# scalar-labs/jepsen

Measured on AMD Instinct MI355X. Metric: history ops verified/sec (node), independent cas-register 10k keys, 1/2/4/8 GPU, higher is better.
Workload: dtype int64

## Files before the change

### include/jh.h

```cpp
#ifndef JH_H
#define JH_H

#include <stddef.h>
#include <stdint.h>

#ifdef __cplusplus
extern "C" {
#endif

#define JH_ABI_VERSION 8

#define JH_OK            0
#define JH_EINVAL        1
#define JH_EUNSUPPORTED  2
#define JH_EDEVICE       3
#define JH_ENOMEM        4

#define JH_TYPE_INVOKE 0
#define JH_TYPE_OK     1
#define JH_TYPE_FAIL   2
#define JH_TYPE_INFO   3

#define JH_F_READ  0
#define JH_F_WRITE 1
// ... 48 lines not shown
#define JH_LIN_INTERN_PER_KEY  4
#define JH_LIN_NO_HELPERS      8
#define JH_LIN_HELPERS_NOW    16
#define JH_LIN_PHASE1_ONLY    32
#define JH_LIN_SKIP_PHASE1    64
#define JH_LIN_NO_HANDOVER   128
#define JH_LIN_STREAM        256
#define JH_LIN_NO_RESUME     512
#define JH_LIN_EXACT_COUNT  1024
#define JH_EXPLORED_UNCOUNTED (-3)
#define JH_LIN_NO_SPEC      2048
#define JH_LIN_SPEC_FIRST   4096
#define JH_LIN_HELP_STALL   8192
#define JH_LIN_NO_TAKEOVER  16384
#define JH_LIN_TAKEOVER     32768

typedef struct jh_lin_opts {
    int64_t init_value;
    int64_t budget;
    int64_t stream;
    int32_t algorithm;
    int32_t flags;
    int64_t quick_budget;
    int64_t phase2_budget;
    int32_t helpers;
    int32_t helper_late_us;
    int32_t xw_waves;
    int32_t p2_waves_per_cu;
    int32_t lean_waves;
    int32_t wide_waves;
    int32_t handover_min;
    int32_t p1_waves_per_cu;
    int32_t bfs_wgs;
    int32_t helper_stall_min;
} jh_lin_opts;

#define JH_DEFAULT_BUDGET (1 << 20)

typedef struct jh_key_verdict {
    int32_t valid;
    int32_t cause;
    int64_t fail_entry;
    int64_t explored;
    int64_t previous_ok;
    int64_t last_op;
    int32_t analyzer;
    int32_t reserved;
} jh_key_verdict;

// ... 29 lines not shown
    int64_t lean_entries;
    int64_t wide_entries;
    int64_t xw_entries;
    int64_t waves[4];
    int64_t streamed;
    int64_t p3_entries;
    double  p2_start_ms;
    double  p1_span_ms;
    int64_t resumed;
    int64_t resume_bytes;
    int64_t spec_jobs;
    int64_t spec_dead;
    int64_t spec_merges;
    int64_t spec_nodes;
    int64_t takeovers;
} jh_summary;

typedef struct jh_ctx jh_ctx;

int  jh_version(void);
int  jh_open(int device, jh_ctx **out);
int  jh_open_multi(int n_gpus, jh_ctx **out);
int  jh_open_devices(const int32_t *devices, int n, jh_ctx **out);
int  jh_n_devices(const jh_ctx *ctx);
void jh_close(jh_ctx *ctx);

int  jh_key_costs(const jh_history *h, int64_t *cost , char *err, size_t errlen);

int jh_check_cas_independent(jh_ctx *ctx, const jh_history *h,
                             const jh_lin_opts *opts,
// ... 258 lines not shown
```

### jepsen_amd/_abi.py

```python
import ctypes as C

JH_ABI_VERSION = 8

JH_OK, JH_EINVAL, JH_EUNSUPPORTED, JH_EDEVICE, JH_ENOMEM = 0, 1, 2, 3, 4
TYPE_INVOKE, TYPE_OK, TYPE_FAIL, TYPE_INFO = 0, 1, 2, 3
F_READ, F_WRITE, F_CAS, F_ADD = 0, 1, 2, 3
F_ENQUEUE, F_DEQUEUE, F_DRAIN = 4, 5, 6
F_FIRST_INTERNED = 16
NIL = -(1 << 63)

VALID, UNKNOWN, INVALID = 0, 1, 2

CAUSES = {
    0: None,
    1: "budget",
    2: "window",
    3: "double-invoke",
    4: "orphan-completion",
    5: "unsupported-f",
    6: "nil-value",
    7: "overflow",
    8: "states",
    9: "deferred",
    10: "multiple-writes",
# ... 25 lines not shown

ALGO_COMPETITION, ALGO_WGL, ALGO_LINEAR = 0, 1, 2
ALGORITHMS = {"competition": ALGO_COMPETITION, "wgl": ALGO_WGL, "linear": ALGO_LINEAR}
LIN_BFS_ONLY, LIN_GEN_JUMP, LIN_INTERN_PER_KEY, LIN_NO_HELPERS, LIN_HELPERS_NOW = 1, 2, 4, 8, 16
LIN_PHASE1_ONLY, LIN_SKIP_PHASE1 = 32, 64
LIN_NO_HANDOVER = 128
LIN_STREAM = 256
LIN_NO_RESUME = 512
LIN_EXACT_COUNT = 1024
EXPLORED_UNCOUNTED = -3
LIN_NO_SPEC = 2048
LIN_SPEC_FIRST = 4096
LIN_HELP_STALL = 8192
LIN_NO_TAKEOVER = 16384
LIN_TAKEOVER = 32768
CAUSE_DEFERRED = 9


class JhLinOpts(C.Structure):
    _fields_ = [("init_value", C.c_int64), ("budget", C.c_int64), ("stream", C.c_int64),
                ("algorithm", C.c_int32), ("flags", C.c_int32),
                ("quick_budget", C.c_int64), ("phase2_budget", C.c_int64),
                ("helpers", C.c_int32), ("helper_late_us", C.c_int32),
                ("xw_waves", C.c_int32), ("p2_waves_per_cu", C.c_int32),
                ("lean_waves", C.c_int32), ("wide_waves", C.c_int32),
                ("handover_min", C.c_int32), ("p1_waves_per_cu", C.c_int32),
                ("bfs_wgs", C.c_int32), ("helper_stall_min", C.c_int32)]


VERDICT_FIELDS = ("valid", "cause", "fail_entry", "explored", "previous_ok", "last_op", "analyzer")
ANALYZER_WGL, ANALYZER_LINEAR = 0, 1
ANALYZERS = {ANALYZER_WGL: "wgl", ANALYZER_LINEAR: "linear"}


class JhKeyVerdict(C.Structure):
    _fields_ = [("valid", C.c_int32), ("cause", C.c_int32),
                ("fail_entry", C.c_int64), ("explored", C.c_int64),
                ("previous_ok", C.c_int64), ("last_op", C.c_int64),
                ("analyzer", C.c_int32), ("reserved", C.c_int32)]


class JhSummary(C.Structure):
    _fields_ = [("valid", C.c_int64), ("n_invalid", C.c_int64), ("n_unknown", C.c_int64),
                ("first_fail_entry", C.c_int64), ("n_keys", C.c_int64),
                ("explored", C.c_int64), ("memo_probes", C.c_int64),
                ("device_ms", C.c_double), ("dfs_ms", C.c_double),
                ("seq_ms", C.c_double), ("bfs_ms", C.c_double), ("n_deferred", C.c_int64),
                ("deferred_entries", C.c_int64), ("seq_probes", C.c_int64),
                ("p3_ms", C.c_double), ("wide_ms", C.c_double), ("xw_ms", C.c_double),
                ("p3_probes", C.c_int64), ("wide_probes", C.c_int64), ("xw_probes", C.c_int64),
                ("helper_probes", C.c_int64), ("n_deferred_wide", C.c_int64), ("n_phase3", C.c_int64),
                ("n_phase3_wide", C.c_int64), ("n_xw", C.c_int64), ("lean_entries", C.c_int64),
                ("wide_entries", C.c_int64), ("xw_entries", C.c_int64), ("waves", C.c_int64 * 4),
                ("streamed", C.c_int64), ("p3_entries", C.c_int64), ("p2_start_ms", C.c_double),
                ("p1_span_ms", C.c_double),
                ("resumed", C.c_int64), ("resume_bytes", C.c_int64),
                ("spec_jobs", C.c_int64), ("spec_dead", C.c_int64), ("spec_merges", C.c_int64),
                ("spec_nodes", C.c_int64), ("takeovers", C.c_int64)]


class JhLinConfig(C.Structure):
    _fields_ = [("key", C.c_int64), ("model_value", C.c_int64), ("n_linearized", C.c_int32),
                ("n_pending", C.c_int32), ("rows_off", C.c_int64),
                ("last_row", C.c_int64)]


CONFIGS_PER_KEY = 10


class JhSetResult(C.Structure):
    _fields_ = [("valid", C.c_int32), ("cause", C.c_int32),
                ("attempt_count", C.c_int64), ("acknowledged_count", C.c_int64),
                ("ok_count", C.c_int64), ("lost_count", C.c_int64),
# ... 187 lines not shown
```

### jepsen_amd/_native.py

```python
import ctypes as C
import os
import threading

import numpy as np

from . import _abi as A

_HERE = os.path.dirname(os.path.abspath(__file__))
LIB_PATH = os.environ.get("JH_LIB") or os.path.join(_HERE, "libjh.so")
_lib = None
_lock = threading.Lock()


class JhError(RuntimeError):
    def __init__(self, code, msg):
        super().__init__(f"libjh error {code}: {msg}")
        self.code = code
        self.msg = msg


def lib():
    global _lib
    with _lock:
        if _lib is None:
# ... 99 lines not shown

def _opts(init, budget, stream=0, algorithm=None, exact_count=True, **tune):
    o = A.JhLinOpts()
    o.init_value = A.NIL if init is None else int(init)
    o.budget = int(budget or 0)
    o.stream = int(stream)
    if isinstance(algorithm, str):
        algorithm = A.ALGORITHMS[algorithm]
    o.algorithm = int(algorithm or 0)
    for k, v in tune.items():
        if k not in dict(A.JhLinOpts._fields_) or k in ("init_value", "budget", "stream", "algorithm", "reserved"):
            raise TypeError(f"unknown jh_lin_opts field {k}")
        setattr(o, k, int(v))
    if exact_count:
        o.flags |= A.LIN_EXACT_COUNT
    return o


def key_costs(cols):
    h = A.make_history(cols)
    out = np.zeros(max(cols.n_keys, 1), dtype=np.int64)
    err = C.create_string_buffer(256)
    rc = lib().jh_key_costs(C.byref(h), out.ctypes.data_as(C.POINTER(C.c_int64)), err, len(err))
    _raise(rc, err)
    return out[:cols.n_keys]


class HostBuffer:

    def __init__(self, count, dtype):
# ... 393 lines not shown
```

### jepsen_amd/csrc/jh_api.hip

```cpp
#include "jh_internal.h"
#include <algorithm>
#include <unordered_map>
#include <vector>

static void set_err(char *err, size_t errlen, const std::string &msg) {
    if (!err || errlen == 0) return;
    size_t k = std::min(errlen - 1, msg.size());
    memcpy(err, msg.data(), k);
    err[k] = 0;
}

template <class F>
static int guarded(char *err, size_t errlen, F &&f) {
    try {
        f();
        set_err(err, errlen, "");
        return JH_OK;
    } catch (const JhException &e) {
        set_err(err, errlen, e.msg);
        return e.code;
    } catch (const std::exception &e) {
        set_err(err, errlen, std::string("internal error: ") + e.what());
        return JH_EDEVICE;
    }
// ... 123 lines not shown
        char e[512] = "";
        int rc = guarded(e, sizeof e, [&] { check_hist(h); });
        if (rc == JH_OK) rc = multi_check_cas_independent(ctx, h, opts, out, sum, e, sizeof e);
        set_err(err, errlen, e);
        return rc;
    }
    std::lock_guard<std::mutex> g(ctx->mu);
    return guarded(err, errlen, [&] {
        check_hist(h);
        HIP_TRY(hipSetDevice(ctx->device));
        hipStream_t st = ctx->stream;
        jh_history d = stage_history(ctx, h, true, false);
        const int64_t K = h->n_keys;
        jh_key_verdict *dv = ctx->ws<jh_key_verdict>(WS_VERDICT, std::max<int64_t>(K, 1));
        if (K == 0) {
            if (sum) { memset(sum, 0, sizeof *sum); sum->first_fail_entry = -1; }
            return;
        }
        lin_check_independent(ctx, &d, opts, true, dv, sum, st);
        HIP_TRY(hipMemcpyAsync(out, dv, sizeof(jh_key_verdict) * K, hipMemcpyDeviceToHost, st));
        HIP_TRY(hipStreamSynchronize(st));
    });
}

int jh_check_cas_independent_device(jh_ctx *ctx, const jh_history *h, const jh_lin_opts *opts,
                                    jh_key_verdict *out_dev, jh_summary *sum, char *err,
                                    size_t errlen) {
    if (!ctx || !out_dev) { set_err(err, errlen, "null context or output"); return JH_EINVAL; }
    ctx = primary(ctx);
    std::lock_guard<std::mutex> g(ctx->mu);
    return guarded(err, errlen, [&] {
        check_hist(h);
        if (!h->on_device) throw_jh(JH_EINVAL, "jh_check_cas_independent_device needs on_device=1");
        HIP_TRY(hipSetDevice(ctx->device));
        hipStream_t st = opts && opts->stream ? (hipStream_t)(intptr_t)opts->stream : ctx->stream;
        if (h->n_keys == 0) {
            if (sum) { memset(sum, 0, sizeof *sum); sum->first_fail_entry = -1; }
            return;
        }
        lin_check_independent(ctx, h, opts, true, out_dev, sum, st);
    });
}

__global__ void k_cfg_slots(const int64_t *__restrict__ keys, int n, int64_t K, int32_t *slot) {
    const int i = blockIdx.x * blockDim.x + threadIdx.x;
    if (i < n && keys[i] >= 0 && keys[i] < K) slot[keys[i]] = i;
}

struct NoopRead { int64_t call, ret; };
static std::vector<std::vector<NoopRead>> noop_reads(const jh_history *h, bool keyed, const int64_t *keys, int nq) {
    const int64_t n = h->n;
    std::vector<int64_t> pr, ty, fc, va, ke;
// ... 397 lines not shown
```

### jepsen_amd/csrc/jh_internal.h

```cpp
#pragma once
#include <hip/hip_runtime.h>
#include <cstdint>
#include <cstdio>
#include <cstdlib>
#include <cstring>
#include <mutex>
#include <thread>
#include <vector>
#include <string>
#include "../../include/jh.h"

#define JH_WAVE 64

struct JhError {
    int code = JH_OK;
    std::string msg;
};

#define HIP_TRY(expr)                                                                 \
    do {                                                                              \
        hipError_t _e = (expr);                                                       \
        if (_e != hipSuccess) {                                                       \
            throw_hip(_e, #expr, __FILE__, __LINE__);                                 \
        }                                                                             \
// ... 86 lines not shown
    WS_SPEC, WS_SPEC_RES, WS_DEBUG_WG, WS_HANDOFF, WS_RS_LOG2,
    WS_U_META, WS_U_PART, WS_U_LIST, WS_U_ALT, WS_U_ALT2, WS_U_BITS, WS_U_TMP, WS_U_FLAG, WS_U_RUNS, WS_U_PAIRS,
    WS_U_CNT, WS_U_IDX, WS_U_SEL, WS_U_OUT,
    WS_B_META, WS_B_WORDS, WS_B_TCNT, WS_B_TBASE, WS_B_TMP, WS_B_ROW, WS_B_START, WS_B_CNT, WS_B_OFF, WS_B_TOT,
    WS_B_BAD, WS_B_CLS, WS_B_FIRST, WS_B_PARTS, WS_B_ACC, WS_B_OUT, WS_B_TRI,
    WS_LF_META, WS_LF_WORDS, WS_LF_TCNT, WS_LF_TBASE, WS_LF_TMP, WS_LF_ROW, WS_LF_START, WS_LF_CNT, WS_LF_GRP, WS_LF_MASK,
    WS_LF_WKEY, WS_LF_WROW, WS_LF_FIRST, WS_LF_KEYS, WS_LF_IDX, WS_LF_RANK, WS_LF_SLOT, WS_LF_CTAB, WS_LF_VTAB, WS_LF_GBITS,
    WS_LF_FLAG, WS_LF_SKEY, WS_LF_SMASK, WS_LF_SROW, WS_LF_PC, WS_LF_OUT,
    WS_CR_META, WS_CR_WORDS, WS_CR_TCNT, WS_CR_TBASE, WS_CR_TMP, WS_CR_WKEY, WS_CR_WVAL, WS_CR_RKEY, WS_CR_RPERM, WS_CR_RROW,
    WS_CR_OFF, WS_CR_TIER, WS_CR_KV, WS_CR_EXP, WS_CR_MISS, WS_CR_SOFF, WS_CR_SCRATCH, WS_CR_OUT, WS_CR_SEG, WS_CR_MBUF,
    WS_CY_META, WS_CY_TMP, WS_CY_PKEY, WS_CY_PROW, WS_CY_COMP, WS_CY_REV, WS_CY_IP, WS_CY_ICOMP, WS_CY_CNT,
    WS_CY_TXN, WS_CY_REC, WS_CY_HASH, WS_CY_HIDX, WS_CY_RAW, WS_CY_EDGES, WS_CY_REACH, WS_CY_BS, WS_CY_REG, WS_CY_SEL,
    WS_CY_FWD, WS_CY_BWD, WS_CY_CSR, WS_CY_STATE, WS_CY_LABEL, WS_CY_SIZE, WS_CY_KEYS, WS_CY_VALS,
    WS_CY_AP_META, WS_CY_AP_ROWS, WS_CY_AP_RECS, WS_CY_AP_LONGEST,
    WS_CY_MO_META, WS_CY_MO_ROWS, WS_CY_MO_RECS,
    WS_COUNT
};

__device__ __forceinline__ uint64_t jh_mix64(uint64_t x) {
    x ^= x >> 33; x *= 0xff51afd7ed558ccdULL;
    x ^= x >> 33; x *= 0xc4ceb9fe1a85ec53ULL;
    x ^= x >> 33; return x;
}

template <class T, class Op>
__device__ __forceinline__ T block_reduce256(T v, Op op, T *sh ) {
    for (int o = 32; o > 0; o >>= 1) v = op(v, (T)__shfl_xor(v, o));
    __syncthreads();
    if ((threadIdx.x & 63) == 0) sh[threadIdx.x >> 6] = v;
    __syncthreads();
// ... 11 lines not shown
    return (int)g;
}

jh_history stage_history(jh_ctx *ctx, const jh_history *h, bool need_key, bool need_aux);
bool ingest_columns(jh_ctx *ctx, const int64_t *const src[7], int64_t *const dst[7], int64_t n, hipStream_t st);
void ingest_free(struct Ingest *g);

struct LinCfgReq {
    const int64_t *keys_dev;
    int32_t n_q, per_key;
    const int32_t *slot_dev;
    jh_lin_config *out_dev;
    int32_t *n_dev;
    int64_t *rows_dev;
};
void lin_check_independent(jh_ctx *ctx, const jh_history *dh, const jh_lin_opts *opts,
                           bool keyed, jh_key_verdict *out_dev, jh_summary *sum,
                           hipStream_t stream, const LinCfgReq *cfg = nullptr);
void key_index(jh_ctx *ctx, const jh_history *dh, int64_t *key_off, int64_t *rows, hipStream_t stream);
void counter_check(jh_ctx *ctx, const jh_history *dh, int64_t *reads_out, int64_t reads_cap,
                   int64_t *n_reads, int64_t *n_errors, int64_t *first_err, int32_t *valid,
                   int32_t *cause, hipStream_t stream);
void set_check(jh_ctx *ctx, const jh_history *dh, jh_set_result *res, int64_t *runs[4],
               int64_t runs_cap, hipStream_t stream);
void set_check_bitmaps(jh_ctx *ctx, const jh_history *dh, jh_set_result *res, uint32_t *bits_out[4],
                       int64_t words_cap, int64_t *base, int64_t *n_words, hipStream_t stream);
void set_full_check(jh_ctx *ctx, const jh_history *dh, const int64_t *time_dev, bool linearizable, int64_t read_batch,
                    jh_set_full_result *res, int64_t *lists_out[3], int64_t list_cap, hipStream_t stream);
void total_queue_check(jh_ctx *ctx, const jh_history *dh, jh_queue_result *res, int64_t *outs[4],
                       int64_t cap, hipStream_t stream);
// ... 33 lines not shown
```

### jepsen_amd/csrc/jh_lin.hip

```cpp
#include "jh_internal.h"
#include <hipcub/hipcub.hpp>
#include <algorithm>
#include <type_traits>
#include "lin/lin_common.h"

namespace {

constexpr int F_READ = 0, F_WRITE = 1, F_CAS = 2, F_OTHER = 4;
constexpr int T_INVOKE = 0, T_OK = 1, T_FAIL = 2, T_INFO = 3;
constexpr uint64_t VIOL_NONE = ~0ULL;
#ifndef JH_LDS_TBL
#define JH_LDS_TBL 0
#endif
constexpr int LDS_TBL = JH_LDS_TBL;
#ifdef JH_STEP_PROF
#define PROF_MARK(v) const unsigned long long v = __builtin_amdgcn_s_memtime()
#define PROF_ADD(acc, a, b) acc += (b) - (a)
#else
#define PROF_MARK(v)
#define PROF_ADD(acc, a, b)
#endif
#ifdef JH_DFS_STATS
#define DFS_STAT(x) x
#else
// ... 334 lines not shown
}
__device__ __forceinline__ bool handover(const DfsArgs &A, uint32_t ins) {
    if (A.handover_min <= 0 || ins < (uint32_t)A.handover_min) return false;
    int q = 0;
    if ((threadIdx.x & 63) == 0) q = __hip_atomic_load(A.queue, __ATOMIC_RELAXED, __HIP_MEMORY_SCOPE_AGENT);
    q = __builtin_amdgcn_readlane(q, 0);
    return q >= (A.n_list_dev ? *A.n_list_dev : A.n_list);
}
constexpr int64_t P2_BUDGET = 1 << 16;
constexpr int64_t QUICK_BUDGET = 8192;
constexpr int32_t HANDOVER_MIN = 1024;
constexpr int32_t P1_PRIO_INS = 0;
constexpr int HELPERS = 64;
constexpr uint64_t HELPER_LATE_US = 250;
constexpr uint32_t HELPER_STALL_MIN = 4096;
constexpr int HELPER_MAINS = 32;

__device__ __forceinline__ bool emit_verdict(jh_key_verdict *out, int32_t *claim, int key,
                                             const jh_key_verdict &v) {
    if (claim && atomicCAS(&claim[key], 0, 1) != 0) return false;
    out[key] = v;
    return true;
}

__device__ __forceinline__ uint64_t ballot(bool b) { return __ballot(b); }
__device__ __forceinline__ int mbcnt(uint64_t m) {
    return __builtin_amdgcn_mbcnt_hi((uint32_t)(m >> 32), __builtin_amdgcn_mbcnt_lo((uint32_t)m, 0));
}
__device__ __forceinline__ int rfl(int x) { return __builtin_amdgcn_readfirstlane(x); }
__device__ __forceinline__ uint32_t rflu(uint32_t x) { return (uint32_t)__builtin_amdgcn_readfirstlane((int)x); }
// ... 3300 lines not shown
    uint32_t *tmp;
    uint64_t *tmpk;
    int32_t linear;
    const int32_t *cfg_slot;
    jh_lin_config *cfg_out;
    int32_t *cfg_n;
    int64_t *cfg_rows;
    int32_t cfg_per;
    const int64_t *col_val, *col_val2;
    int64_t vmin, init_value;
    int32_t per_key_values;
    const int32_t *live_n;
    const int32_t *p1_done, *p1_tot;
    unsigned long long *t_span;
    unsigned long long *tl;
};

struct BfsShared {
    KeyInfo K;
    jh_key_verdict v;
    int key, need, maxw, status, mode, gclear, ovf, term;
    unsigned npend, npend2, nfront, nnext, tmax, lcount, r;
    unsigned nnodes, nostore, dlen, clen, cnext, ok;
    unsigned fbase;
    unsigned long long count, ccount, plen;
    alignas(16) uint32_t win_vv[64];
    uint32_t win_f[64];
    unsigned long long cfg_min;
    unsigned gl_cnt[2], gl_ovf[2];
};

static_assert(sizeof(BfsShared) <= BFS_HDR, "BFS header");

__device__ __forceinline__ uint64_t bfs_pack(uint32_t t, uint32_t s, uint32_t m) {
    return ((uint64_t)t << 44) | ((uint64_t)s << 32) | m;
}
__device__ __forceinline__ uint32_t lset_hash(uint64_t k) {
    uint32_t h = (uint32_t)k * 0x9E3779B1u ^ (uint32_t)(k >> 32) * 0x85EBCA77u;
    h ^= h >> 16;
    h *= 0x7FEB352Du;
    return (h >> 11) & (LSET - 1);
}

__device__ __forceinline__ int bfs_child(const Op *ops, const int32_t *woff, const uint16_t *W, const uint8_t *rpos,
// ... 1091 lines not shown
        if (tid == 0) {
            jh_key_verdict v;
            v.valid = JH_UNKNOWN; v.cause = JH_CAUSE_BUDGET; v.fail_entry = -1; v.explored = A.budget;
            emit_verdict(A.out, A.claim, key, v);
        }
    } else if (wid == 0) {
        jh_key_verdict v;
        v.valid = JH_INVALID; v.cause = 0;
        v.explored = (int64_t)sh.count - 1;
        v.fail_entry = ret_row(A.src, K, sh.tmax, lane);
        if (lane == 0) emit_verdict(A.out, A.claim, key, v);
    }
    __syncthreads();
}

__global__ void __launch_bounds__(BFS_THREADS) k_lin_bfs(BfsArgs A0) {
    BfsShared &sh = *(BfsShared *)jh_lds;
    BfsArgs A = A0;
    A.nodes += (size_t)blockIdx.x * A.ncap;
    A.lstart += (size_t)blockIdx.x * A.lcap;
    A.ent += (size_t)blockIdx.x * A.hcap;
    A.slot += (size_t)blockIdx.x * A.ncap;
    A.vis += (size_t)blockIdx.x * (A.ncap / 32 + 1);
    A.tmp += (size_t)blockIdx.x * A.ncap;
    A.tmpk += (size_t)blockIdx.x * A.ncap;
    const int tid = threadIdx.x, lane = tid & 63, wid = tid >> 6;
    uint64_t *gset = A.gset + (size_t)blockIdx.x * A.gset_cap;
    uint64_t *pend = A.pend + (size_t)blockIdx.x * 2 * A.q_cap;
    uint64_t *front = A.front + (size_t)blockIdx.x * 2 * A.q_cap;
    char *gscr = A.scratch + (size_t)blockIdx.x * A.scratch_bytes;
    bool spanned = false;
    for (;;) {
        if (tid == 0) {
            const int idx = atomicAdd(A.queue, 1);
            if (A.live_n) sh.key = stream_key(A.list, A.live_n, A.p1_done, A.p1_tot, idx, A.src.flags);
            else sh.key = idx < A.n_list ? A.list[idx] : -1;
        }
        __syncthreads();
        const int key = sh.key;
        if (key < 0) break;
        if (A.t_span && !spanned && tid == 0) atomicMin(&A.t_span[0], __builtin_amdgcn_s_memrealtime());
        spanned = true;
        TL_REC(A.tl, key, 0);
        if (wid == 0) {
            KeyInfo K;
            jh_key_verdict v;
            const bool need = key_pass1(A.src, key, lane, K, v);
            if (lane == 0) { sh.K = K; sh.v = v; sh.need = need; }
        }
        __syncthreads();
        if (!sh.need) {
            if (tid == 0) emit_verdict(A.out, A.claim, key, sh.v);
            if (wid == 0 && A.cfg_slot && A.cfg_slot[key] >= 0 && sh.v.valid == JH_VALID && sh.v.explored == 0 &&
// ... 924 lines not shown
    void phase1_tables();
    void phase1_args();
    void phase1_resume();
    void phase2_budgets();
    void ensure_lds_attrs();
    void prep_xw(const int32_t *qw);
    void prep_wide();
    void launch_wide(hipStream_t sw, bool p2);
    WgArgs build_wg(int wg_cus, int32_t *wg_claim, int32_t *wg_queue, bool all_cus = false);
    void prep_race(int nd_all, int nd_l);
    void race_bfs(int nd_all);
    int race_helper_count(int nd_l);
    uint64_t *race_lean_sizing(int nd_l, int help_cus);
    void race_helpers(int nd_l);
    void race_lean_args(int nd_l, uint64_t *memo2);
    void timeline_tables(bool wide);
    DfsArgs phase1_wide_args() const;
    DfsArgs phase3_lean_args() const;
    DfsArgs phase3_wide_args() const;
    void launch_phase3_lean(int waves, hipStream_t s);
    void entry_lists(bool live);
    void record_no_heavy_keys();
    void run_streaming();
    void run_phase1();
    void sort_deferred();
    void run_stage1();
    void launch_xw();
    void run_wg_mode();
    void run_linear();
    void run_race();
// ... 419 lines not shown
    const uint32_t set_cap = sz.set_cap, q_cap = sz.q_cap;
    uint32_t hcap = 1u << 16;
    while (hcap < 2 * (uint64_t)ncap) hcap <<= 1;
    const uint32_t lcap = (uint32_t)smax + 2;
    const int bfs_cus = std::max(1, nd_all > 2000 && nd_all <= 4000 ? ctx->n_cu / 4
                                                                      : std::min(96, ctx->n_cu * 3 / 8));
    wg2 = std::min(nd_all, tune_env("JH_BFS_CUS") ? std::max(1, atoi(tune_env("JH_BFS_CUS"))) :
                           opts && opts->bfs_wgs > 0 ? std::min(opts->bfs_wgs, ctx->n_cu - 16) : bfs_cus);
    const uint64_t per_bfs = (uint64_t)set_cap * 8 + 4ULL * q_cap * 8 + scr_bytes_bfs + (uint64_t)ncap * 8 +
                             (uint64_t)lcap * 4 + (uint64_t)hcap * 16 + (uint64_t)ncap * 4 + ((uint64_t)ncap / 32 + 1) * 4 +
                             (uint64_t)ncap * 4 + (uint64_t)ncap * 8;
    wg2 = fit_units(ctx, wg2, per_bfs, {WS_BFS_SET, WS_BFS_Q, WS_BFS_NODES, WS_BFS_HKEY, WS_BFS_TMPK});
    uint64_t *bset = ctx->ws<uint64_t>(WS_BFS_SET, (size_t)wg2 * set_cap);
    uint64_t *bq = ctx->ws<uint64_t>(WS_BFS_Q, (size_t)wg2 * 4 * q_cap);
    char *bscr = ctx->ws<char>(WS_SCRATCH_BFS, (size_t)wg2 * scr_bytes_bfs);
    int32_t *unres = ctx->ws<int32_t>(WS_BFS_META, nd_all + 1);
    c = BfsArgs{};
    c.src = key_src();
    c.list = defer; c.n_list = nd_all; c.queue = q + Q_QUEUE; c.out = out_dev;
    c.unres_list = unres; c.unres_count = q + Q_UNRES;
    c.gset = bset; c.gset_cap = set_cap; c.pend = bq; c.front = bq + (size_t)wg2 * 2 * q_cap;
    c.q_cap = q_cap;
    c.scratch = bscr; c.scratch_bytes = scr_bytes_bfs; c.budget = budget;
    c.init_state = init_state; c.states_ok = n_states < 4096 ? 1 : 0;
    c.dbg = dbg; c.claim = claim;
    c.reach_cap = reach_cap;
    bfs_only = (lflags & JH_LIN_BFS_ONLY) != 0;
    c.dbg_plen = tune_env("JH_BFS_DBGV") && atoi(tune_env("JH_BFS_DBGV")) ? 1 : 0;
    c.exact_count = (lflags & JH_LIN_EXACT_COUNT) || c.dbg_plen ? 1 : 0;
    c.ncap = ncap; c.hcap = hcap; c.lcap = lcap;
    c.nodes = ctx->ws<uint64_t>(WS_BFS_NODES, (size_t)wg2 * ncap);
// ... 111 lines not shown
    b.dbg = dbg ? dbg + 16 * 256 : nullptr; b.claim = claim;
    b.probes = (unsigned long long *)(q + Q_PROBES_SEQ);
    b.seq_start = seq_start; b.exit_count = seq_start ? q + Q_SEQ_EXIT : nullptr;
    b.stamp_progress = seq_start && (lflags & JH_LIN_HELP_STALL) ? 1 : 0;
    b.stall = seq_stall;
    b.defer_time = nullptr;
    b.handoff = nullptr;
    if (n_help > 0 && a.rs_off && waves2 > 0 && (lflags & JH_LIN_TAKEOVER) && !(lflags & JH_LIN_NO_TAKEOVER)) {
        int32_t *ho = ctx->ws<int32_t>(WS_HANDOFF, K);
        HIP_TRY(hipMemsetAsync(ho, 0, (size_t)K * sizeof(int32_t), st));
        b.handoff = ho;
        b.hlog_cap = 32768;
        b.hlog = ctx->ws<uint32_t>(WS_RS_LOG2, (size_t)wmax * b.hlog_cap);
        wh.d.handoff = ho;
    }
}

void LinRun::timeline_tables(bool wide) {
    if (!defer_times) return;
    unsigned long long *tl = ctx->ws<unsigned long long>(WS_TL, TL_W * (size_t)K);
    HIP_TRY(hipMemsetAsync(tl, 0, TL_W * sizeof(unsigned long long) * K, st));
    c.tl = tl; b.tl = tl;
    if (wide) bw.tl = tl;
    if (n_help > 0) wh.d.tl = tl;
}

DfsArgs LinRun::phase1_wide_args() const {
    DfsArgs aw = a;
    aw.list = list_w; aw.n_list_dev = q + Q_N_LIST_W; aw.queue = q + Q_P1W_QUEUE;
    aw.defer_kind = d64 + 2 * (K + 1); aw.defer_kind_count = q + Q_DEFER_W;
// ... 325 lines not shown
            xa.cfg_slot = cfgreq->slot_dev; xa.cfg_out = cfgreq->out_dev; xa.cfg_n = cfgreq->n_dev;
            xa.cfg_rows = cfgreq->rows_dev; xa.cfg_per = cfgreq->per_key;
            xa.col_val = dh->value; xa.col_val2 = dh->value2;
            xa.vmin = vmin; xa.init_value = init; xa.per_key_values = per_key_values ? 1 : 0;
            k_lin_xw<<<waves_x, 64, 0, st>>>(xa);
            HIP_TRY(hipGetLastError());
        }
        n_x = 0;
    }
    HIP_TRY(hipEventRecord(ctx->ev[EV_P2_END], st));
    HIP_TRY(hipEventRecord(ctx->ev[EV_SEQ_END], st));
}

void LinRun::run_race() {
    prep_race(n_defer, n_def_l);
    if (resume) b.rs_mode = 2;
    if (!resume) { b.handoff = nullptr; wh.d.handoff = nullptr; }
    timeline_tables(true);

    prep_wide();
    HIP_TRY(hipEventRecord(ctx->ev[EV_FORK], st));
    HIP_TRY(hipStreamWaitEvent(ctx->aux, ctx->ev[EV_FORK], 0));
    k_lin_bfs<<<wg2, BFS_THREADS, BFS_LDS_BYTES, st>>>(c);
    HIP_TRY(hipGetLastError());
    HIP_TRY(hipEventRecord(ctx->ev[EV_BFS_END], st));
    bool wide_done = bfs_only;
    if (bfs_only || (waves2 == 0 && waves_w == 0)) {}
    else if (wg_race) { if (waves2) k_lin_wg<<<n_wg, WG_THREADS, WG_LDS, ctx->aux>>>(wr); }
    else if (p2_m) {
        DfsPair pr;
// ... 67 lines not shown
    sum->n_keys = sh[4]; sum->explored = sh[5];
    sum->memo_probes = q64(qh, Q_PROBES_P1);
    float ms = 0, ms_dfs = 0;
    HIP_TRY(hipEventElapsedTime(&ms, ctx->ev[EV_START], ctx->ev[EV_END]));
    HIP_TRY(hipEventElapsedTime(&ms_dfs, ctx->ev[EV_P1_START], ctx->ev[EV_P1_END]));
    sum->device_ms = ms; sum->dfs_ms = ms_dfs;
    sum->n_deferred = n_defer;
    sum->deferred_entries = q64(qh, Q_ENT_ALL);
    sum->seq_probes = q64(qh, Q_PROBES_SEQ);
    sum->seq_ms = 0; sum->bfs_ms = 0; sum->p3_ms = 0; sum->wide_ms = 0; sum->xw_ms = 0;
    sum->streamed = stream_p2 ? 1 : 0;
    sum->p3_entries = q64(qh, Q_ENT_P3);
    sum->p2_start_ms = -1; sum->p1_span_ms = 0;
    sum->resumed = resume ? qh[Q_RS_PUBLISHED] : 0;
    sum->takeovers = resume ? qh[Q_RS_TAKEOVERS] : 0;
    sum->spec_nodes = q64(qh, Q_SPEC); sum->spec_merges = qh[Q_SPEC_MERGES];
    sum->spec_jobs = qh[Q_SPEC_JOBS]; sum->spec_dead = qh[Q_SPEC_DEAD];
    sum->resume_bytes = resume ? q64(qh, Q_RS_USED) : 0;
    if (stream_p2) {
        sum->p1_span_ms = span_ms(qh, Q_T_P1);
        sum->seq_ms = span_ms(qh, Q_T_LEAN);
        sum->bfs_ms = span_ms(qh, Q_T_BFS);
        sum->xw_ms = span_ms(qh, Q_T_XW);
        if (waves_w > 0) sum->wide_ms = span_ms(qh, Q_T_WIDE);
        if (split3) { float c2 = 0; HIP_TRY(hipEventElapsedTime(&c2, ctx->ev[EV_P3_START], ctx->ev[EV_SEQ_END])); sum->p3_ms = c2; }
        const int64_t p1s = q64(qh, Q_T_P1);
        int64_t first = -1;
        for (int w : {Q_T_BFS, Q_T_LEAN}) {
            const int64_t t = q64(qh, w);
            if (t != -1 && (first == -1 || t < first)) first = t;
// ... 95 lines not shown
```

### jepsen_amd/csrc/jh_multi.hip

```cpp
#include "jh_internal.h"
#include <algorithm>
#include <queue>
#include <mutex>
#include <thread>

namespace {

int host_threads() {
    unsigned n = std::thread::hardware_concurrency();
    return (int)std::max(1u, std::min(n, 16u));
}

void key_costs_host(const jh_history *h, int64_t *cost) {
    const int64_t N = h->n, K = h->n_keys;
    std::fill(cost, cost + K, 0);
    if (N == 0 || K == 0 || !h->key) return;
    const int T = host_threads();
    const int64_t chunk = (N + T - 1) / T;
    std::vector<int64_t> cnt((size_t)T * T, 0);
    auto run = [&](auto &&fn) {
        std::vector<std::thread> th;
        for (int t = 0; t < T; ++t) th.emplace_back(fn, t);
        for (auto &x : th) x.join();
    };
// ... 191 lines not shown
    const int n = (int)g->members.size();
    if (h->on_device) {
        snprintf(err, errlen, "a multi-device context takes host columns (on_device=0)");
        return JH_EUNSUPPORTED;
    }
    const int64_t K = h->n_keys, N = h->n;
    std::vector<int64_t> cost(K);
    std::vector<SubHist> sub(n);
    try {
        key_costs_host(h, cost.data());
        split(h, assign_lpt(cost.data(), K, n), n, sub);
    } catch (const std::exception &e) {
        snprintf(err, errlen, "multi-device split: %s", e.what());
        return JH_ENOMEM;
    }
    jh_lin_opts o = opts ? *opts : jh_lin_opts{JH_NIL, 0, 0};
    o.stream = 0;
    const bool two_stage = o.algorithm != JH_ALGO_LINEAR && !(o.flags & (JH_LIN_PHASE1_ONLY | JH_LIN_SKIP_PHASE1));
    jh_lin_opts o1 = o;
    if (two_stage) o1.flags |= JH_LIN_PHASE1_ONLY;
    std::vector<std::vector<jh_key_verdict>> v(n);
    std::vector<jh_summary> s(n);
    std::vector<int> rc(n, JH_OK);
    std::vector<std::string> msg(n);
    MultiStats st{std::vector<double>(n, 0.0), std::vector<int64_t>(n, 0)};
    {
        std::vector<std::thread> th;
        for (int d = 0; d < n; ++d)
            th.emplace_back([&, d] {
                jh_history sh = sub_view(sub[d]);
                v[d].resize(std::max<int64_t>(1, sh.n_keys));
// ... 69 lines not shown
                    }
                    jh_history sh = sub_view(S);
                    std::vector<jh_key_verdict> vv(std::max<int64_t>(1, sh.n_keys));
                    jh_summary ss;
                    char e[512];
                    const int r = jh_check_cas_independent(g->members[d], &sh, &o2, vv.data(), &ss, e, sizeof e);
                    std::lock_guard<std::mutex> lk(mu);
                    if (r != JH_OK) { rc[d] = r; msg[d] = e; return; }
                    place(S, vv);
                    st.ms[d] += ss.device_ms;
                    st.keys2[d] += (int64_t)(b - a);
                    s[d].seq_probes += ss.seq_probes; s[d].p3_probes += ss.p3_probes;
                    s[d].wide_probes += ss.wide_probes; s[d].helper_probes += ss.helper_probes;
                    s[d].seq_ms += ss.seq_ms; s[d].bfs_ms += ss.bfs_ms; s[d].wide_ms += ss.wide_ms;
                    s[d].p3_ms += ss.p3_ms; s[d].n_phase3 += ss.n_phase3; s[d].n_phase3_wide += ss.n_phase3_wide;
                }
            });
        for (auto &x : th) x.join();
        for (int d = 0; d < n; ++d)
            if (rc[d] != JH_OK) {
                snprintf(err, errlen, "device %d (stage 2): %s", d, msg[d].c_str());
                return rc[d];
            }
    }
    jh_summary m{};
    m.first_fail_entry = -1;
    for (int64_t k = 0; k < K; ++k) {
        const jh_key_verdict &x = out[k];
        if (x.explored < 0) continue;
        m.n_keys++;
// ... 7 lines not shown
        if (x.valid == JH_UNKNOWN) m.n_unknown++;
    }
    for (int d = 0; d < n; ++d) {
        const jh_summary &a = s[d];
        m.memo_probes += a.memo_probes;
        m.n_deferred += a.n_deferred; m.deferred_entries += a.deferred_entries; m.seq_probes += a.seq_probes;
        m.device_ms = std::max(m.device_ms, st.ms[d]);
        m.dfs_ms = std::max(m.dfs_ms, a.dfs_ms);
        m.seq_ms = std::max(m.seq_ms, a.seq_ms);
        m.bfs_ms = std::max(m.bfs_ms, a.bfs_ms);
        m.p3_ms = std::max(m.p3_ms, a.p3_ms);
        m.wide_ms = std::max(m.wide_ms, a.wide_ms);
        m.xw_ms = std::max(m.xw_ms, a.xw_ms);
        m.p3_probes += a.p3_probes; m.wide_probes += a.wide_probes; m.xw_probes += a.xw_probes;
        m.helper_probes += a.helper_probes; m.n_deferred_wide += a.n_deferred_wide;
        m.n_phase3 += a.n_phase3; m.n_phase3_wide += a.n_phase3_wide; m.n_xw += a.n_xw;
        m.lean_entries += a.lean_entries; m.wide_entries += a.wide_entries; m.xw_entries += a.xw_entries;
        for (int i = 0; i < 4; i++) m.waves[i] = std::max(m.waves[i], a.waves[i]);
    }
    if (sum) *sum = m;
    if (err && errlen) err[0] = 0;
    return JH_OK;
}
```

### jepsen_amd/csrc/lin/lin_common.h

```cpp
#pragma once

namespace {

constexpr int Q_WORDS = 104;
constexpr int Q_QUEUE = 0, Q_DEFER = 1, Q_FLAGS = 2, Q_UNRES = 3, Q_PROBES_P1 = 4;
constexpr int Q_P2_QUEUE = 6, Q_WIDE_QUEUE = 7, Q_PROBES_SEQ = 8, Q_BUMP = 10;
constexpr int Q_N_LIST = 12, Q_N_LIST_W = 13, Q_P1W_QUEUE = 14;
constexpr int Q_DEFER3 = 16, Q_P3_QUEUE_FEW = 17, Q_P3_QUEUE = 18, Q_N_LIST_X = 19, Q_P3W_QUEUE = 20;
constexpr int Q_XW_QUEUE = 21, Q_PROBES_XW = 22, Q_XW_MAX = 26, Q_SEQ_EXIT = 28;
constexpr int Q_ENT_ALL = 24, Q_DEFER_L = 29, Q_DEFER_W = 30, Q_DEFER3W = 31;
constexpr int Q_PROBES_HELP = 32, Q_PROBES_P3 = 34, Q_PROBES_WIDE = 36;
constexpr int Q_ENT_LEAN = 40, Q_ENT_WIDE = 42, Q_ENT_XW = 44;
constexpr int Q_T_WIDE = 46;
constexpr int Q_T_END = 2;
constexpr int Q_P1_DONE = 64, Q_SEQ_WAVES = 65, Q_BFS_QUEUE = 66;
constexpr int Q_T_BFS = 68, Q_T_LEAN = 72, Q_T_XW = 76, Q_T_P1 = 80;
constexpr int Q_ENT_P3 = 84;
constexpr int Q_RS_USED = 88;
constexpr int Q_RS_PUBLISHED = 90, Q_RS_TAKEOVERS = 91;
constexpr int Q_MAINS = 92;
constexpr int Q_SPEC = 96;
constexpr int Q_SPEC_MERGES = 98, Q_SPEC_JOBS = 99, Q_SPEC_DEAD = 100;
constexpr int QF_TABLE_OVERFLOW = 2;
constexpr int QF_STACK_OVERFLOW = 4;
constexpr int QF_LOST_ITEM = 16, QF_IDLE_ENUM = 32, QF_FULL_SET = 64, QF_STEP_LIMIT = 128;
constexpr int QF_BAD_WINDOW = 256;
constexpr int QF_STREAM_WAIT = 512;
constexpr int QF_WG_WATCHDOGS = 0x1F0;
constexpr int QF_WATCHDOGS = 0x3F0;

constexpr int V_HANDED = -9;
constexpr int32_t HO_NONE = 0, HO_ASK = 1, HO_DONE = 2, HO_REFUSED = 3, HO_WITHDRAWN = 4, HO_SAVING = 5;

}
```

Measured before the change: 259.4 million.

## Let BFS workgroups pick stalled sequential keys during race phase

```diff
diff --git a/include/jh.h b/include/jh.h
--- a/include/jh.h
+++ b/include/jh.h
@@ -86,6 +86,7 @@
 #define JH_LIN_HELP_STALL   8192
 #define JH_LIN_NO_TAKEOVER  16384
 #define JH_LIN_TAKEOVER     32768
+#define JH_LIN_TAIL_FIELDS  65536
 
 typedef struct jh_lin_opts {
     int64_t init_value;
@@ -105,6 +106,8 @@
     int32_t p1_waves_per_cu;
     int32_t bfs_wgs;
     int32_t helper_stall_min;
+    int32_t bfs_stall_min;
+    int32_t reserved;
 } jh_lin_opts;
 
 #define JH_DEFAULT_BUDGET (1 << 20)
@@ -164,6 +167,7 @@
     int64_t spec_merges;
     int64_t spec_nodes;
     int64_t takeovers;
+    int64_t bfs_stall_picks;
 } jh_summary;
 
 typedef struct jh_ctx jh_ctx;
diff --git a/jepsen_amd/_abi.py b/jepsen_amd/_abi.py
--- a/jepsen_amd/_abi.py
+++ b/jepsen_amd/_abi.py
@@ -63,6 +63,7 @@
 LIN_HELP_STALL = 8192
 LIN_NO_TAKEOVER = 16384
 LIN_TAKEOVER = 32768
+LIN_TAIL_FIELDS = 65536
 CAUSE_DEFERRED = 9
 
 
@@ -74,7 +75,8 @@
                 ("xw_waves", C.c_int32), ("p2_waves_per_cu", C.c_int32),
                 ("lean_waves", C.c_int32), ("wide_waves", C.c_int32),
                 ("handover_min", C.c_int32), ("p1_waves_per_cu", C.c_int32),
-                ("bfs_wgs", C.c_int32), ("helper_stall_min", C.c_int32)]
+                ("bfs_wgs", C.c_int32), ("helper_stall_min", C.c_int32),
+                ("bfs_stall_min", C.c_int32), ("reserved", C.c_int32)]
 
 
 VERDICT_FIELDS = ("valid", "cause", "fail_entry", "explored", "previous_ok", "last_op", "analyzer")
@@ -105,7 +107,8 @@
                 ("p1_span_ms", C.c_double),
                 ("resumed", C.c_int64), ("resume_bytes", C.c_int64),
                 ("spec_jobs", C.c_int64), ("spec_dead", C.c_int64), ("spec_merges", C.c_int64),
-                ("spec_nodes", C.c_int64), ("takeovers", C.c_int64)]
+                ("spec_nodes", C.c_int64), ("takeovers", C.c_int64),
+                ("bfs_stall_picks", C.c_int64)]
 
 
 class JhLinConfig(C.Structure):
diff --git a/jepsen_amd/_native.py b/jepsen_amd/_native.py
--- a/jepsen_amd/_native.py
+++ b/jepsen_amd/_native.py
@@ -137,6 +137,7 @@
         setattr(o, k, int(v))
     if exact_count:
         o.flags |= A.LIN_EXACT_COUNT
+    o.flags |= A.LIN_TAIL_FIELDS
     return o
 
 
diff --git a/jepsen_amd/csrc/jh_api.hip b/jepsen_amd/csrc/jh_api.hip
--- a/jepsen_amd/csrc/jh_api.hip
+++ b/jepsen_amd/csrc/jh_api.hip
@@ -161,7 +161,7 @@
         const int64_t K = h->n_keys;
         jh_key_verdict *dv = ctx->ws<jh_key_verdict>(WS_VERDICT, std::max<int64_t>(K, 1));
         if (K == 0) {
-            if (sum) { memset(sum, 0, sizeof *sum); sum->first_fail_entry = -1; }
+            if (sum) { memset(sum, 0, lin_summary_bytes(opts)); sum->first_fail_entry = -1; }
             return;
         }
         lin_check_independent(ctx, &d, opts, true, dv, sum, st);
@@ -182,7 +182,7 @@
         HIP_TRY(hipSetDevice(ctx->device));
         hipStream_t st = opts && opts->stream ? (hipStream_t)(intptr_t)opts->stream : ctx->stream;
         if (h->n_keys == 0) {
-            if (sum) { memset(sum, 0, sizeof *sum); sum->first_fail_entry = -1; }
+            if (sum) { memset(sum, 0, lin_summary_bytes(opts)); sum->first_fail_entry = -1; }
             return;
         }
         lin_check_independent(ctx, h, opts, true, out_dev, sum, st);
diff --git a/jepsen_amd/csrc/jh_internal.h b/jepsen_amd/csrc/jh_internal.h
--- a/jepsen_amd/csrc/jh_internal.h
+++ b/jepsen_amd/csrc/jh_internal.h
@@ -124,6 +124,7 @@
     WS_CY_FWD, WS_CY_BWD, WS_CY_CSR, WS_CY_STATE, WS_CY_LABEL, WS_CY_SIZE, WS_CY_KEYS, WS_CY_VALS,
     WS_CY_AP_META, WS_CY_AP_ROWS, WS_CY_AP_RECS, WS_CY_AP_LONGEST,
     WS_CY_MO_META, WS_CY_MO_ROWS, WS_CY_MO_RECS,
+    WS_BFS_TAKEN,
     WS_COUNT
 };
 
@@ -165,6 +166,12 @@
     int32_t *n_dev;
     int64_t *rows_dev;
 };
+inline size_t lin_opts_bytes(const jh_lin_opts *o) {
+    return o && (o->flags & JH_LIN_TAIL_FIELDS) ? sizeof(jh_lin_opts) : offsetof(jh_lin_opts, bfs_stall_min);
+}
+inline size_t lin_summary_bytes(const jh_lin_opts *o) {
+    return o && (o->flags & JH_LIN_TAIL_FIELDS) ? sizeof(jh_summary) : offsetof(jh_summary, bfs_stall_picks);
+}
 void lin_check_independent(jh_ctx *ctx, const jh_history *dh, const jh_lin_opts *opts,
                            bool keyed, jh_key_verdict *out_dev, jh_summary *sum,
                            hipStream_t stream, const LinCfgReq *cfg = nullptr);
diff --git a/jepsen_amd/csrc/jh_lin.hip b/jepsen_amd/csrc/jh_lin.hip
--- a/jepsen_amd/csrc/jh_lin.hip
+++ b/jepsen_amd/csrc/jh_lin.hip
@@ -372,6 +372,7 @@
 constexpr int HELPERS = 64;
 constexpr uint64_t HELPER_LATE_US = 250;
 constexpr uint32_t HELPER_STALL_MIN = 4096;
+constexpr uint32_t BFS_STALL_MIN = 4096;
 constexpr int HELPER_MAINS = 32;
 
 __device__ __forceinline__ bool emit_verdict(jh_key_verdict *out, int32_t *claim, int key,
@@ -3702,7 +3703,19 @@
     const int32_t *p1_done, *p1_tot;
     unsigned long long *t_span;
     unsigned long long *tl;
+    const struct BfsPick *pk;
 };
+
+struct BfsPick {
+    const uint32_t *stall;
+    int32_t *taken;
+    const int32_t *seq_queue;
+    const int32_t *seq_exit;
+    int32_t *picked;
+    uint32_t stall_min;
+    int32_t seq_n, seq_waves;
+};
+__global__ void k_bfs_pick_args(BfsPick *dst, BfsPick v) { *dst = v; }
 
 struct BfsShared {
     KeyInfo K;
@@ -3716,6 +3729,10 @@
     uint32_t win_f[64];
     unsigned long long cfg_min;
     unsigned gl_cnt[2], gl_ovf[2];
+    unsigned long long pick;
+    unsigned long long t_enter;
+    int open;
+    int list_done;
 };
 
 static_assert(sizeof(BfsShared) <= BFS_HDR, "BFS header");
@@ -4837,6 +4854,54 @@
     __syncthreads();
 }
 
+constexpr unsigned long long BFS_WAIT_MAX_TICKS = 500000000ULL;
+__device__ __attribute__((noinline)) void bfs_pick(const BfsArgs &A, BfsShared &sh, int tid) {
+    const BfsPick &P = *A.pk;
+    for (;;) {
+        if (tid == 0) { sh.pick = 0; sh.open = 0; }
+        __syncthreads();
+        for (int i = tid; i < A.n_list; i += BFS_THREADS) {
+            const int key = A.list[i];
+            if (__hip_atomic_load(&A.claim[key], __ATOMIC_RELAXED, __HIP_MEMORY_SCOPE_AGENT)) continue;
+            sh.open = 1;
+            const uint32_t stl = __hip_atomic_load(&P.stall[key], __ATOMIC_RELAXED, __HIP_MEMORY_SCOPE_AGENT);
+            if (stl < P.stall_min || __hip_atomic_load(&P.taken[key], __ATOMIC_RELAXED, __HIP_MEMORY_SCOPE_AGENT))
+                continue;
+            atomicMax(&sh.pick, ((unsigned long long)stl << 24) | (unsigned long long)(0xFFFFFF - i));
+        }
+        __syncthreads();
+        if (tid == 0) {
+            int k = -2;
+            const bool late = __builtin_amdgcn_s_memrealtime() - sh.t_enter > BFS_WAIT_MAX_TICKS;
+            bool done = sh.list_done != 0;
+            if (sh.pick) {
+                const int key = A.list[0xFFFFFF - (int)(sh.pick & 0xFFFFFF)];
+                if (atomicCAS(&P.taken[key], 0, 1) == 0) { k = key; atomicAdd(P.picked, 1); }
+                else k = -3;
+            } else if (late || ld_agent(P.seq_queue) >= P.seq_n) {
+                while (!done) {
+                    const int idx = atomicAdd(A.queue, 1);
+                    if (idx >= A.n_list) { done = true; break; }
+                    const int key = A.list[idx];
+                    if (__hip_atomic_load(&A.claim[key], __ATOMIC_RELAXED, __HIP_MEMORY_SCOPE_AGENT) ||
+                        __hip_atomic_load(&P.taken[key], __ATOMIC_RELAXED, __HIP_MEMORY_SCOPE_AGENT))
+                        continue;
+                    k = key;
+                    break;
+                }
+                sh.list_done = done;
+                if (k < 0 && done && (!sh.open || late || ld_agent(P.seq_exit) >= P.seq_waves)) k = -1;
+            }
+            sh.key = k;
+        }
+        __syncthreads();
+        const int k = sh.key;
+        if (k >= 0 || k == -1) return;
+        if (k == -2)
+            for (int j = 0; j < 16; j++) __builtin_amdgcn_s_sleep(127);
+    }
+}
+
 __global__ void __launch_bounds__(BFS_THREADS) k_lin_bfs(BfsArgs A0) {
     BfsShared &sh = *(BfsShared *)jh_lds;
     BfsArgs A = A0;
@@ -4853,13 +4918,18 @@
     uint64_t *front = A.front + (size_t)blockIdx.x * 2 * A.q_cap;
     char *gscr = A.scratch + (size_t)blockIdx.x * A.scratch_bytes;
     bool spanned = false;
+    if (A.pk && tid == 0) { sh.t_enter = __builtin_amdgcn_s_memrealtime(); sh.list_done = 0; }
     for (;;) {
-        if (tid == 0) {
-            const int idx = atomicAdd(A.queue, 1);
-            if (A.live_n) sh.key = stream_key(A.list, A.live_n, A.p1_done, A.p1_tot, idx, A.src.flags);
-            else sh.key = idx < A.n_list ? A.list[idx] : -1;
-        }
-        __syncthreads();
+        if (A.pk) {
+            bfs_pick(A, sh, tid);
+        } else {
+            if (tid == 0) {
+                const int idx = atomicAdd(A.queue, 1);
+                if (A.live_n) sh.key = stream_key(A.list, A.live_n, A.p1_done, A.p1_tot, idx, A.src.flags);
+                else sh.key = idx < A.n_list ? A.list[idx] : -1;
+            }
+            __syncthreads();
+        }
         const int key = sh.key;
         if (key < 0) break;
         if (A.t_span && !spanned && tid == 0) atomicMin(&A.t_span[0], __builtin_amdgcn_s_memrealtime());
@@ -5814,6 +5884,7 @@
     uint64_t *race_lean_sizing(int nd_l, int help_cus);
     void race_helpers(int nd_l);
     void race_lean_args(int nd_l, uint64_t *memo2);
+    void race_bfs_pick(int nd_l);
     void timeline_tables(bool wide);
     DfsArgs phase1_wide_args() const;
     DfsArgs phase3_lean_args() const;
@@ -6263,7 +6334,7 @@
     uint64_t *bset = ctx->ws<uint64_t>(WS_BFS_SET, (size_t)wg2 * set_cap);
     uint64_t *bq = ctx->ws<uint64_t>(WS_BFS_Q, (size_t)wg2 * 4 * q_cap);
     char *bscr = ctx->ws<char>(WS_SCRATCH_BFS, (size_t)wg2 * scr_bytes_bfs);
-    int32_t *unres = ctx->ws<int32_t>(WS_BFS_META, nd_all + 1);
+    int32_t *unres = ctx->ws<int32_t>(WS_BFS_META, 2 * (size_t)nd_all + 1);
     c = BfsArgs{};
     c.src = key_src();
     c.list = defer; c.n_list = nd_all; c.queue = q + Q_QUEUE; c.out = out_dev;
@@ -6405,6 +6476,28 @@
         b.hlog = ctx->ws<uint32_t>(WS_RS_LOG2, (size_t)wmax * b.hlog_cap);
         wh.d.handoff = ho;
     }
+}
+
+void LinRun::race_bfs_pick(int nd_l) {
+    if (bfs_only || wg_race || waves2 <= 0 || nd_l <= 0) return;
+    int32_t *buf = ctx->ws<int32_t>(WS_BFS_TAKEN, 32 + 2 * (size_t)K);
+    static_assert(sizeof(BfsPick) <= 32 * sizeof(int32_t), "BfsPick");
+    int32_t *taken = buf + 32;
+    HIP_TRY(hipMemsetAsync(taken, 0, (seq_stall ? 1 : 2) * (size_t)K * sizeof(int32_t), st));
+    if (!seq_stall) seq_stall = (uint32_t *)(taken + K);
+    b.stall = seq_stall;
+    b.exit_count = q + Q_SEQ_EXIT;
+    BfsPick pk{};
+    pk.stall = seq_stall;
+    pk.stall_min = opts && (opts->flags & JH_LIN_TAIL_FIELDS) && opts->bfs_stall_min > 0 ? (uint32_t)opts->bfs_stall_min
+                                                                                       : BFS_STALL_MIN;
+    pk.taken = taken;
+    pk.seq_queue = q + Q_P2_QUEUE; pk.seq_n = nd_l;
+    pk.seq_exit = q + Q_SEQ_EXIT; pk.seq_waves = waves2;
+    pk.picked = q + Q_BFS_PICKS;
+    k_bfs_pick_args<<<1, 1, 0, st>>>((BfsPick *)buf, pk);
+    HIP_TRY(hipGetLastError());
+    c.pk = (const BfsPick *)buf;
 }
 
 void LinRun::timeline_tables(bool wide) {
@@ -6760,6 +6853,7 @@
 
 void LinRun::run_race() {
     prep_race(n_defer, n_def_l);
+    race_bfs_pick(n_def_l);
     if (resume) b.rs_mode = 2;
     if (!resume) { b.handoff = nullptr; wh.d.handoff = nullptr; }
     timeline_tables(true);
@@ -6857,6 +6951,7 @@
     sum->p2_start_ms = -1; sum->p1_span_ms = 0;
     sum->resumed = resume ? qh[Q_RS_PUBLISHED] : 0;
     sum->takeovers = resume ? qh[Q_RS_TAKEOVERS] : 0;
+    if (opts && (opts->flags & JH_LIN_TAIL_FIELDS)) sum->bfs_stall_picks = qh[Q_BFS_PICKS];
     sum->spec_nodes = q64(qh, Q_SPEC); sum->spec_merges = qh[Q_SPEC_MERGES];
     sum->spec_jobs = qh[Q_SPEC_JOBS]; sum->spec_dead = qh[Q_SPEC_DEAD];
     sum->resume_bytes = resume ? q64(qh, Q_RS_USED) : 0;
diff --git a/jepsen_amd/csrc/jh_multi.hip b/jepsen_amd/csrc/jh_multi.hip
--- a/jepsen_amd/csrc/jh_multi.hip
+++ b/jepsen_amd/csrc/jh_multi.hip
@@ -229,7 +229,8 @@
         snprintf(err, errlen, "multi-device split: %s", e.what());
         return JH_ENOMEM;
     }
-    jh_lin_opts o = opts ? *opts : jh_lin_opts{JH_NIL, 0, 0};
+    jh_lin_opts o{JH_NIL, 0, 0};
+    if (opts) memcpy(&o, opts, lin_opts_bytes(opts));
     o.stream = 0;
     const bool two_stage = o.algorithm != JH_ALGO_LINEAR && !(o.flags & (JH_LIN_PHASE1_ONLY | JH_LIN_SKIP_PHASE1));
     jh_lin_opts o1 = o;
@@ -329,6 +330,7 @@
                     s[d].wide_probes += ss.wide_probes; s[d].helper_probes += ss.helper_probes;
                     s[d].seq_ms += ss.seq_ms; s[d].bfs_ms += ss.bfs_ms; s[d].wide_ms += ss.wide_ms;
                     s[d].p3_ms += ss.p3_ms; s[d].n_phase3 += ss.n_phase3; s[d].n_phase3_wide += ss.n_phase3_wide;
+                    if (o2.flags & JH_LIN_TAIL_FIELDS) s[d].bfs_stall_picks += ss.bfs_stall_picks;
                 }
             });
         for (auto &x : th) x.join();
@@ -366,11 +368,12 @@
         m.xw_ms = std::max(m.xw_ms, a.xw_ms);
         m.p3_probes += a.p3_probes; m.wide_probes += a.wide_probes; m.xw_probes += a.xw_probes;
         m.helper_probes += a.helper_probes; m.n_deferred_wide += a.n_deferred_wide;
+        if (o.flags & JH_LIN_TAIL_FIELDS) m.bfs_stall_picks += a.bfs_stall_picks;
         m.n_phase3 += a.n_phase3; m.n_phase3_wide += a.n_phase3_wide; m.n_xw += a.n_xw;
         m.lean_entries += a.lean_entries; m.wide_entries += a.wide_entries; m.xw_entries += a.xw_entries;
         for (int i = 0; i < 4; i++) m.waves[i] = std::max(m.waves[i], a.waves[i]);
     }
-    if (sum) *sum = m;
+    if (sum) memcpy(sum, &m, lin_summary_bytes(&o));
     if (err && errlen) err[0] = 0;
     return JH_OK;
 }
diff --git a/jepsen_amd/csrc/lin/lin_common.h b/jepsen_amd/csrc/lin/lin_common.h
--- a/jepsen_amd/csrc/lin/lin_common.h
+++ b/jepsen_amd/csrc/lin/lin_common.h
@@ -19,6 +19,7 @@
 constexpr int Q_RS_USED = 88;
 constexpr int Q_RS_PUBLISHED = 90, Q_RS_TAKEOVERS = 91;
 constexpr int Q_MAINS = 92;
+constexpr int Q_BFS_PICKS = 93;
 constexpr int Q_SPEC = 96;
 constexpr int Q_SPEC_MERGES = 98, Q_SPEC_JOBS = 99, Q_SPEC_DEAD = 100;
 constexpr int QF_TABLE_OVERFLOW = 2;
```

Measured after the change: 265.5 million, median of 6. +2.4%, better.
